# c-zhou/oatk

Hardware: AMD Instinct MI355X
Metric: HiFi Gbases/s through syncasm (syncmer+syncerr) at k=1001 s=31 (higher is better)
Workload: dtype u64

## Files before the change

oatk_amd/csrc/api.hip:

```cpp
#include <hip/hip_runtime.h>
#include <rocprim/device/device_radix_sort.hpp>
#include <rocprim/device/device_scan.hpp>
#include <rocprim/device/device_transform.hpp>
#include <stdio.h>
#include <stdlib.h>
#include <string.h>
#include <time.h>
#include <execinfo.h>
#include <sys/mman.h>
#include <condition_variable>
#include <mutex>
#include <string>
#include <thread>
#include <utility>
#include <vector>

#include "../../include/oatk_hip.h"
#include "common.hpp"
#include "scan_hpc.hpp"
#include "scan_syncmer.hpp"
#include "scan_syncmer_fast.hpp"
#include "kmer_hash.hpp"
#include "count.hpp"

// ... 412 lines not shown
oatk_hip_ctx *oatk_hip_create(int device)
{
    int n = 0;
    if (hipGetDeviceCount(&n) != hipSuccess || device < 0 || device >= n) return nullptr;
    if (hipSetDevice(device) != hipSuccess) return nullptr;
    oatk_hip_ctx *ctx = new oatk_hip_ctx();
    ctx->device = device;
    { int cu = 0; if (hipDeviceGetAttribute(&cu, hipDeviceAttributeMultiprocessorCount, device) == hipSuccess && cu > 0) ctx->n_cu = cu; }
    if (hipStreamCreateWithFlags(&ctx->stream, hipStreamNonBlocking) != hipSuccess) { delete ctx; return nullptr; }
    for (int i = 0; i <= OATK_T_COUNT_; ++i) {
        (void) hipEventCreate(&ctx->ev[i][0]);
        (void) hipEventCreate(&ctx->ev[i][1]);
        ctx->ev_used[i] = false;
    }
    memset(ctx->ms, 0, sizeof(ctx->ms));
    return ctx;
}

void oatk_hip_destroy(oatk_hip_ctx *ctx)
{
    if (!ctx) return;
    (void) hipSetDevice(ctx->device);
    (void) hipStreamSynchronize(ctx->stream);
    DevBuf *all[] = {&ctx->in_seq, &ctx->in_off, &ctx->in_len, &ctx->hoco_l, &ctx->n_scm, &ctx->n_nn, &ctx->n_lrl, &ctx->ho_rl,
                     &ctx->hoco_s, &ctx->nbits, &ctx->nn_key, &ctx->lrl_key, &ctx->lrl_val, &ctx->nn_key2, &ctx->lrl_key2,
                     &ctx->lrl_val2, &ctx->raw_lo, &ctx->raw_smer, &ctx->raw_mpos, &ctx->shard_cnt, &ctx->counters, &ctx->n_scm64,
                     &ctx->scm_off, &ctx->pos_hash, &ctx->pos_lo, &ctx->pos_smer, &ctx->pos_mpos, &ctx->pos_kid, &ctx->key_hash,
                     &ctx->key_sorted, &ctx->iota, &ctx->perm, &ctx->head, &ctx->head_idx, &ctx->newclus, &ctx->clus_id, &ctx->kloc, &ctx->smer_sorted, &ctx->slot_rec, &ctx->scm_loc,
                     &ctx->bad_head, &ctx->tag, &ctx->tmp_perm, &ctx->flags, &ctx->scm_h, &ctx->scm_s, &ctx->scm_cov,
                     &ctx->scm_occ_off, &ctx->scm_occ, &ctx->tmp};
    for (DevBuf *b : all) b->release();
    ec_state_free(ctx);
    cons_state_free(ctx);
    ing_state_free(ctx);
    stat_state_free(ctx);
    ag_state_free(ctx);
    ovl_state_free(ctx);
    ra_state_free(ctx);
    rc_state_free(ctx);
    multi_state_free(ctx);
    for (int i = 0; i <= OATK_T_COUNT_; ++i) {
        (void) hipEventDestroy(ctx->ev[i][0]);
        (void) hipEventDestroy(ctx->ev[i][1]);
    }
    staging_free(ctx);
    (void) hipStreamDestroy(ctx->stream);
    delete ctx;
}

int oatk_hip_mem_pool(oatk_hip_ctx *ctx, uint64_t warm_bytes)
{
    if (!ctx) return OATK_E_NODEV;
    { const char *e = getenv("OATK_POOL"); if (e && e[0] == '0') return OATK_OK; }
    CK(hipSetDevice(ctx->device));
    if (ctx->device < 0 || ctx->device >= 64) return OATK_E_ARG;
    ChunkPool *pl;
    {
        std::unique_lock<std::mutex> lk(g_pool_mu);
        pl = g_pool[ctx->device];
        if (!pl) {
            int vmm = 0;
            if (hipDeviceGetAttribute(&vmm, hipDeviceAttributeVirtualMemoryManagementSupported, ctx->device) != hipSuccess || !vmm) { (void) hipGetLastError(); return OATK_OK; }
            pl = new ChunkPool();
            pl->device = ctx->device;
            memset(&pl->prop, 0, sizeof(pl->prop));
            pl->prop.type = hipMemAllocationTypePinned;
            pl->prop.location.type = hipMemLocationTypeDevice;
            pl->prop.location.id = ctx->device;
            memset(&pl->acc, 0, sizeof(pl->acc));
            pl->acc.location = pl->prop.location;
            pl->acc.flags = hipMemAccessFlagsProtReadWrite;
            static bool at_exit = false;
            if (!at_exit) { at_exit = true; atexit(pools_end); }
            pl->on = true;
            g_pool[ctx->device] = pl;
        }
    }
    if (warm_bytes) pl->warm((size_t) warm_bytes);
    return OATK_OK;
}

const char *oatk_hip_last_error(oatk_hip_ctx *ctx) { return ctx? ctx->err.c_str() : "no device context"; }
void *oatk_hip_stream(oatk_hip_ctx *ctx) { return ctx? (void *) ctx->stream : nullptr; }
int oatk_hip_sync(oatk_hip_ctx *ctx)
{
    if (!ctx) return OATK_E_NODEV;
    CK(hipStreamSynchronize(ctx->stream));
    return OATK_OK;
}
int oatk_hip_set_timing(oatk_hip_ctx *ctx, int enable)
{
    if (!ctx) return OATK_E_NODEV;
    ctx->timing = enable != 0;
    return OATK_OK;
}
int oatk_hip_get_timing(oatk_hip_ctx *ctx, float *ms, int n)
{
    if (!ctx) return OATK_E_NODEV;
    for (int i = 0; i < n && i < OATK_T_COUNT_; ++i) ms[i] = ctx->ms[i];
    return OATK_OK;
}
int oatk_hip_debug_force_general(oatk_hip_ctx *ctx, int on)
{
    if (!ctx) return OATK_E_NODEV;
    ctx->force_general = on != 0;
    return OATK_OK;
}
int oatk_hip_debug_align_two_pass(oatk_hip_ctx *ctx, int on)
{
    if (!ctx) return OATK_E_NODEV;
    ctx->ra_two_pass = on != 0;
    return OATK_OK;
}
int oatk_hip_debug_list_cap(oatk_hip_ctx *ctx, int cap)
{
    if (!ctx) return OATK_E_NODEV;
    if (cap < 0 || cap > oatk::SYF_LIST) { ctx->err = "oatk_hip_debug_list_cap: 0 <= cap <= 128"; return OATK_E_ARG; }
    ctx->list_cap = cap;
    return OATK_OK;
}
int oatk_hip_debug_hash_mask(oatk_hip_ctx *ctx, uint64_t mask)
{
    if (!ctx) return OATK_E_NODEV;
    ctx->hash_mask = mask;
    return OATK_OK;
}

__global__ void widen_kernel(const uint32_t *in, uint64_t *out, uint64_t n)
{
    uint64_t i = (uint64_t) blockIdx.x * blockDim.x + threadIdx.x;
    if (i < n) out[i] = in[i];
    if (i == n) out[i] = 0;
}

static void scan_reset_downstream(oatk_hip_ctx *ctx);

static int launch_scan_kernels(oatk_hip_ctx *ctx)
{
    using namespace oatk;
    const uint64_t n = ctx->n_reads;
    CK(hipMemsetAsync(ctx->counters.p, 0, 4 * sizeof(uint32_t), ctx->stream));
    CK(hipMemsetAsync(ctx->shard_cnt.p, 0, oatk::OATK_REC_SHARDS * sizeof(uint32_t), ctx->stream));
    HpcArgs h;
    h.seq = ctx->d_seq, h.off = ctx->d_off, h.len = ctx->d_len, h.sid0 = ctx->sid0;
    h.ho_rl = ctx->ho_rl.as<uint8_t>(), h.hoco_s = ctx->hoco_s.as<uint8_t>(), h.nbits = ctx->nbits.as<uint32_t>();
    h.hoco_l = ctx->hoco_l.as<uint32_t>(), h.n_nn = ctx->n_nn.as<uint32_t>(), h.n_lrl = ctx->n_lrl.as<uint32_t>();
    h.nn_key = ctx->nn_key.as<uint64_t>(), h.lrl_key = ctx->lrl_key.as<uint64_t>(), h.lrl_val = ctx->lrl_val.as<uint32_t>();
    h.nn_cap = ctx->nn_cap, h.lrl_cap = ctx->lrl_cap, h.counters = ctx->counters.as<uint32_t>();
    t_begin(ctx, OATK_T_HPC);
    h.n_reads = (uint32_t) n;
    constexpr int HPC_NW = 4;
    uint64_t hpc_grid = (uint64_t) ctx->n_cu * 8 * 8;
    { const char *ev = getenv("OATK_DEBUG_HPC_GRID"); if (ev && atoi(ev) > 0) hpc_grid = (uint64_t) atoi(ev); }
    if (hpc_grid * HPC_NW > n) hpc_grid = (n + HPC_NW - 1) / HPC_NW;
    unsigned hpc_dyn = 0;
    { const char *ev = getenv("OATK_DEBUG_HPC_LDS"); if (ev && atoi(ev) > 0) hpc_dyn = (unsigned) atoi(ev); }
    hipLaunchKernelGGL((hpc_pack_kernel<HPC_NW>), dim3((unsigned) (hpc_grid? hpc_grid : 1)), dim3(HPC_NW * OATK_WAVE), hpc_dyn, ctx->stream, h);
    t_end(ctx, OATK_T_HPC);

    SynArgs s;
    s.hoco_s = ctx->hoco_s.as<uint8_t>(), s.nbits = ctx->nbits.as<uint32_t>(), s.off = ctx->d_off;
    s.hoco_l = ctx->hoco_l.as<uint32_t>(), s.n_nn = ctx->n_nn.as<uint32_t>(), s.sid0 = ctx->sid0;
    s.K = ctx->K, s.S = ctx->S, s.want_n = 0, s.n_scm = ctx->n_scm.as<uint32_t>(), s.list_cap = ctx->list_cap? ctx->list_cap : SYF_LIST;
    s.rec_hash = nullptr, s.rec_lo = ctx->raw_lo.as<uint64_t>(), s.rec_smer = ctx->raw_smer.as<uint64_t>();
    s.rec_mpos = ctx->raw_mpos.as<uint32_t>(), s.region_cap = ctx->region_cap, s.shard_cnt = ctx->shard_cnt.as<uint32_t>();
    const bool small = ctx->K + 8 * SYN_NT + 8 + 64 <= 4096;
    const int fast_ring = ctx->force_general? 0 : syncmer_fast_ring(ctx->K, ctx->S);
    t_begin(ctx, OATK_T_SYNCMER);
    if (fast_ring == 4096) {
        const dim3 g((unsigned) n), b(SYN_NT);
        unsigned dyn = 0;
        { const char *ev = getenv("OATK_DEBUG_SYNCMER_LDS"); if (ev && atoi(ev) > 0) dyn = (unsigned) atoi(ev); }
#define OATK_SYF_SWITCH(S31) switch ((-(ctx->K - ctx->S)) & 7) { \
            case 0: OATK_SYF_LAUNCH(S31, 0); break; case 1: OATK_SYF_LAUNCH(S31, 1); break; case 2: OATK_SYF_LAUNCH(S31, 2); break; \
            case 3: OATK_SYF_LAUNCH(S31, 3); break; case 4: OATK_SYF_LAUNCH(S31, 4); break; case 5: OATK_SYF_LAUNCH(S31, 5); break; \
            case 6: OATK_SYF_LAUNCH(S31, 6); break; default: OATK_SYF_LAUNCH(S31, 7); break; }
        const bool two_waves = ctx->K - ctx->S < 1024 && getenv("OATK_DEBUG_SYNCMER_NT256") == nullptr;
#define OATK_SYF_LAUNCH(S31, SH) do { if (two_waves) hipLaunchKernelGGL((syncmer_fast_kernel<2048, S31, 128, SH>), g, dim3(128), dyn, ctx->stream, s); \
                                      else hipLaunchKernelGGL((syncmer_fast_kernel<4096, S31, SYN_NT, SH>), g, b, dyn, ctx->stream, s); } while (0)
        if (ctx->S == 31) OATK_SYF_SWITCH(true) else OATK_SYF_SWITCH(false)
#undef OATK_SYF_SWITCH
#undef OATK_SYF_LAUNCH
    }
    else if (small) hipLaunchKernelGGL((syncmer_kernel<8, 4096, false>), dim3((unsigned) n), dim3(SYN_NT), 0, ctx->stream, s);
    else hipLaunchKernelGGL((syncmer_kernel<16, 8192, false>), dim3((unsigned) n), dim3(SYN_NT), 0, ctx->stream, s);
    t_end(ctx, OATK_T_SYNCMER);
    uint32_t n_amb = 0;
    CK(hipMemcpyAsync(&n_amb, ctx->counters.as<uint32_t>(), 4, hipMemcpyDeviceToHost, ctx->stream));
    CK(hipStreamSynchronize(ctx->stream));
    s.want_n = 1;
    t_begin(ctx, OATK_T_SYNCMER_N);
    if (n_amb) {
        if (small) hipLaunchKernelGGL((syncmer_kernel<8, 4096, true>), dim3((unsigned) n), dim3(SYN_NT), 0, ctx->stream, s);
        else hipLaunchKernelGGL((syncmer_kernel<16, 8192, true>), dim3((unsigned) n), dim3(SYN_NT), 0, ctx->stream, s);
    }
    t_end(ctx, OATK_T_SYNCMER_N);
    CK(hipGetLastError());
    return OATK_OK;
}

int oatk_hip_scan(oatk_hip_ctx *ctx, const uint8_t *d_seq, const uint64_t *d_off, const uint32_t *d_len,
                  uint64_t n_reads, uint64_t seq_bytes, uint64_t sid0, int k, int s)
{
    if (!ctx) return OATK_E_NODEV;
    CK(hipSetDevice(ctx->device));
    if (!(s > 0 && s < 32 && k > s) || k > oatk_hip_max_k()) { ctx->err = "k/s out of range for the device scan"; return OATK_E_ARG; }
    if (seq_bytes % OATK_READ_ALIGN || n_reads >= 0xFFFFFFFFULL || sid0 + n_reads > 0xFFFFFFFFULL) { ctx->err = "bad batch geometry"; return OATK_E_ARG; }
    ctx->d_seq = d_seq, ctx->d_off = d_off, ctx->d_len = d_len;
    ctx->n_reads = n_reads, ctx->seq_bytes = seq_bytes, ctx->sid0 = sid0, ctx->K = k, ctx->S = s;
    scan_reset_downstream(ctx);
    ctx->retries = 0, ctx->collisions = 0;
    ctx->n_occ = ctx->tot_nn = ctx->tot_lrl = ctx->n_scm_total = 0;
    if (n_reads == 0) { ctx->scanned = true; return OATK_OK; }

    ENSURE(hoco_l, n_reads * 4); ENSURE(n_scm, n_reads * 4); ENSURE(n_nn, n_reads * 4); ENSURE(n_lrl, n_reads * 4);
    ENSURE(ho_rl, seq_bytes + 64);
    ENSURE(hoco_s, seq_bytes / 4 + 128 + 16 + ctx->import_reserve);
    ENSURE(nbits, seq_bytes / 8 + 128, true);
    ENSURE(counters, 64);
    if (ctx->nn_cap == 0) ctx->nn_cap = 1u << 14;
    if (ctx->lrl_cap == 0) ctx->lrl_cap = 1u << 14;
    const uint32_t NSH = oatk::OATK_REC_SHARDS;
    {
        uint64_t guess = (seq_bytes / 256 + 1024) / NSH + 256;
        if (ctx->region_cap < guess) ctx->region_cap = (uint32_t) guess;
    }
    ENSURE(shard_cnt, NSH * 4);
    uint32_t sc[oatk::OATK_REC_SHARDS];
    uint32_t sc_max = 0;

    for (;;) {
        const size_t raw_n = (size_t) ctx->region_cap * NSH;
        ENSURE(raw_lo, raw_n * 8); ENSURE(raw_smer, raw_n * 8); ENSURE(raw_mpos, raw_n * 4);
        ENSURE(nn_key, (size_t) ctx->nn_cap * 8); ENSURE(nn_key2, (size_t) ctx->nn_cap * 8);
        ENSURE(lrl_key, (size_t) ctx->lrl_cap * 8); ENSURE(lrl_key2, (size_t) ctx->lrl_cap * 8);
        ENSURE(lrl_val, (size_t) ctx->lrl_cap * 4); ENSURE(lrl_val2, (size_t) ctx->lrl_cap * 4);
        int rc = launch_scan_kernels(ctx);
        if (rc) return rc;
        uint32_t c[4];
        CK(hipMemcpyAsync(c, ctx->counters.p, sizeof(c), hipMemcpyDeviceToHost, ctx->stream));
        CK(hipMemcpyAsync(sc, ctx->shard_cnt.p, sizeof(sc), hipMemcpyDeviceToHost, ctx->stream));
        CK(hipStreamSynchronize(ctx->stream));
        bool again = false;
        if (c[0] > ctx->nn_cap) ctx->nn_cap = c[0] + c[0] / 4, again = true;
        if (c[1] > ctx->lrl_cap) ctx->lrl_cap = c[1] + c[1] / 4, again = true;
        uint64_t tot = 0;
        uint32_t mx = 0;
        for (uint32_t i = 0; i < NSH; ++i) { tot += sc[i]; if (sc[i] > mx) mx = sc[i]; }
        sc_max = mx;
        if (mx > ctx->region_cap) ctx->region_cap = mx + mx / 4 + 16, again = true;
        if (tot > 0xFFFFFFF0ULL) { ctx->err = "more than 2^32 syncmer occurrences in one batch"; return OATK_E_ARG; }
        ctx->tot_nn = c[0], ctx->tot_lrl = c[1], ctx->n_occ = tot;
        if (!again) break;
        ++ctx->retries;
        CK(hipMemsetAsync(ctx->nbits.p, 0, ctx->nbits.cap, ctx->stream));
    }
    if (ctx->timing) t_collect(ctx, OATK_T_HPC, OATK_T_SYNCMER_N);

    t_begin(ctx, OATK_T_SCAN_POST);
    ctx->nn_sorted_in_2 = ctx->lrl_sorted_in_2 = false;
    if (ctx->tot_nn > 1) {
        size_t tb = 0;
        CK(rocprim::radix_sort_keys(nullptr, tb, ctx->nn_key.as<uint64_t>(), ctx->nn_key2.as<uint64_t>(), ctx->tot_nn, 0, 64, ctx->stream));
        ENSURE(tmp, tb);
        CK(rocprim::radix_sort_keys(ctx->tmp.p, tb, ctx->nn_key.as<uint64_t>(), ctx->nn_key2.as<uint64_t>(), ctx->tot_nn, 0, 64, ctx->stream));
        ctx->nn_sorted_in_2 = true;
    }
    if (ctx->tot_lrl > 1) {
        size_t tb = 0;
        CK(rocprim::radix_sort_pairs(nullptr, tb, ctx->lrl_key.as<uint64_t>(), ctx->lrl_key2.as<uint64_t>(), ctx->lrl_val.as<uint32_t>(),
                                     ctx->lrl_val2.as<uint32_t>(), ctx->tot_lrl, 0, 64, ctx->stream));
        ENSURE(tmp, tb);
        CK(rocprim::radix_sort_pairs(ctx->tmp.p, tb, ctx->lrl_key.as<uint64_t>(), ctx->lrl_key2.as<uint64_t>(), ctx->lrl_val.as<uint32_t>(),
                                     ctx->lrl_val2.as<uint32_t>(), ctx->tot_lrl, 0, 64, ctx->stream));
        ctx->lrl_sorted_in_2 = true;
    }
    {
        ENSURE(n_scm64, (n_reads + 1) * 8); ENSURE(scm_off, (n_reads + 1) * 8);
        unsigned nb = (unsigned) ((n_reads + 1 + 255) / 256);
        hipLaunchKernelGGL(widen_kernel, dim3(nb), dim3(256), 0, ctx->stream, ctx->n_scm.as<uint32_t>(), ctx->n_scm64.as<uint64_t>(), n_reads);
        size_t tb = 0;
        CK(rocprim::exclusive_scan(nullptr, tb, ctx->n_scm64.as<uint64_t>(), ctx->scm_off.as<uint64_t>(), (uint64_t) 0, n_reads + 1,
                                   rocprim::plus<uint64_t>(), ctx->stream));
        ENSURE(tmp, tb);
        CK(rocprim::exclusive_scan(ctx->tmp.p, tb, ctx->n_scm64.as<uint64_t>(), ctx->scm_off.as<uint64_t>(), (uint64_t) 0, n_reads + 1,
                                   rocprim::plus<uint64_t>(), ctx->stream));
    }
    t_end(ctx, OATK_T_SCAN_POST);

    {
        size_t n = ctx->n_occ? ctx->n_occ : 1;
        ENSURE(pos_hash, n * 8); ENSURE(pos_lo, n * 8); ENSURE(pos_smer, n * 8); ENSURE(pos_mpos, n * 4);
        ENSURE(key_hash, n * 8); ENSURE(iota, n * 4); ENSURE(slot_rec, n * 32);
    }
    if (ctx->n_occ) {
        oatk::KmerHashArgs kh;
        kh.hoco_s = ctx->hoco_s.as<uint8_t>(), kh.off = ctx->d_off, kh.sid0 = ctx->sid0;
        kh.raw_lo = ctx->raw_lo.as<uint64_t>(), kh.raw_smer = ctx->raw_smer.as<uint64_t>(), kh.raw_mpos = ctx->raw_mpos.as<uint32_t>();
        kh.shard_cnt = ctx->shard_cnt.as<uint32_t>(), kh.region_cap = ctx->region_cap;
        kh.scm_off = ctx->scm_off.as<uint64_t>(), kh.hash_mask = ctx->hash_mask;
        kh.pos_hash = ctx->pos_hash.as<uint64_t>(), kh.pos_lo = ctx->pos_lo.as<uint64_t>(), kh.pos_smer = ctx->pos_smer.as<uint64_t>();
        kh.pos_mpos = ctx->pos_mpos.as<uint32_t>(), kh.key_hash = ctx->key_hash.as<uint64_t>(), kh.iota = ctx->iota.as<uint32_t>();
        kh.slot_rec = ctx->slot_rec.as<uint4>(), kh.K = ctx->K;
        const int nw = ((ctx->K - 1) / 4 + 1 + 7) / 8;
        t_begin(ctx, OATK_T_KMER_HASH);
        hipLaunchKernelGGL(oatk::kmer_hash_kernel, dim3((sc_max + KMH_REC - 1) / KMH_REC, NSH), dim3(64), (size_t) KMH_REC * (nw + 1) * 8, ctx->stream, kh);
        t_end(ctx, OATK_T_KMER_HASH);
    }
    CK(hipGetLastError());
    CK(hipStreamSynchronize(ctx->stream));
    if (ctx->timing) { t_collect(ctx, OATK_T_SCAN_POST, OATK_T_COUNT_PLACE); t_collect(ctx, OATK_T_KMER_HASH, OATK_T_KMER_HASH); }
    ctx->scanned = true;
    ctx->slots_packed = ctx->n_occ != 0;
    return OATK_OK;
}

__global__ void append_rebase_kernel(const uint64_t *src, uint64_t *dst, uint64_t n, uint64_t add)
{
    uint64_t i = (uint64_t) blockIdx.x * blockDim.x + threadIdx.x;
    if (i < n) dst[i] = src[i] + add;
}
__global__ void append_iota_kernel(uint32_t *iota, uint64_t first, uint64_t n)
{
    uint64_t i = (uint64_t) blockIdx.x * blockDim.x + threadIdx.x;
    if (i < n) iota[first + i] = (uint32_t) (first + i);
}

static void scan_reset_downstream(oatk_hip_ctx *ctx)
{
    ctx->scanned = ctx->counted = false;
    ctx->slots_packed = false;
    if (ctx->ec) ctx->ec->done = ctx->ec->marked = ctx->ec->graph_resident = ctx->ec->global = false;
    if (ctx->cons) ctx->cons->done = false;
    if (ctx->ag) ctx->ag->done = false;
    if (ctx->ovl) ctx->ovl->done = false;
    if (ctx->ra) ctx->ra->done = false;
    if (ctx->multi) ctx->multi->merged = ctx->multi->ec_done = false;
}

int oatk_hip_device(oatk_hip_ctx *ctx) { return ctx? ctx->device : -1; }

int oatk_hip_d2d(oatk_hip_ctx *ctx, void *d_dst, const void *d_src, uint64_t bytes)
{
    if (!ctx) return OATK_E_NODEV;
    if (bytes == 0) return OATK_OK;
    CK(hipSetDevice(ctx->device));
    CK(hipMemcpyAsync(d_dst, d_src, bytes, hipMemcpyDeviceToDevice, ctx->stream));
    CK(hipStreamSynchronize(ctx->stream));
    return OATK_OK;
}

int oatk_hip_scan_begin(oatk_hip_ctx *ctx, uint64_t sid0, int k, int s)
{
    if (!ctx) return OATK_E_NODEV;
    CK(hipSetDevice(ctx->device));
    if (!(s > 0 && s < 32 && k > s) || k > oatk_hip_max_k()) { ctx->err = "k/s out of range for the device scan"; return OATK_E_ARG; }
    scan_reset_downstream(ctx);
    ctx->d_seq = nullptr, ctx->d_off = nullptr, ctx->d_len = nullptr;
    ctx->n_reads = 0, ctx->seq_bytes = 0, ctx->sid0 = sid0, ctx->K = k, ctx->S = s;
    ctx->retries = 0, ctx->collisions = 0;
    ctx->n_occ = ctx->tot_nn = ctx->tot_lrl = ctx->n_scm_total = 0;
    ctx->nn_sorted_in_2 = ctx->lrl_sorted_in_2 = false;
    ctx->scanned = true;
    return OATK_OK;
}

#define KEEP(buf, bytes, used)                                                                     \
    do {                                                                                           \
        if (!ctx->buf.grow_keep((bytes), (used), ctx->stream)) {                                   \
            ctx->err = "hipMalloc failed for " #buf " (append)";                                   \
            return OATK_E_NOMEM;                                                                   \
        }                                                                                          \
    } while (0)

static int append_ensure(oatk_hip_ctx *ctx, uint64_t nr, uint64_t sb, uint64_t occ, uint64_t nn, uint64_t lrl)
{
    const uint64_t n0 = ctx->n_reads, b0 = ctx->seq_bytes, o0 = ctx->n_occ;
    KEEP(in_off, (nr + 1) * 8, n0 * 8);
    KEEP(hoco_l, nr * 4 + 4, n0 * 4); KEEP(n_scm, nr * 4 + 4, n0 * 4); KEEP(n_nn, nr * 4 + 4, n0 * 4); KEEP(n_lrl, nr * 4 + 4, n0 * 4);
    KEEP(ho_rl, sb + 64, b0);
    KEEP(hoco_s, sb / 4 + 128 + 16 + ctx->import_reserve, b0 / 4 + 64);
    KEEP(scm_off, (nr + 1) * 8, (n0 + 1) * 8);
    KEEP(pos_hash, occ * 8 + 8, o0 * 8); KEEP(pos_lo, occ * 8 + 8, o0 * 8); KEEP(pos_smer, occ * 8 + 8, o0 * 8); KEEP(pos_mpos, occ * 4 + 4, o0 * 4);
    KEEP(key_hash, occ * 8 + 8, o0 * 8); KEEP(iota, occ * 4 + 4, o0 * 4);
    KEEP(nn_key, nn * 8 + 8, ctx->tot_nn * 8); KEEP(lrl_key, lrl * 8 + 8, ctx->tot_lrl * 8); KEEP(lrl_val, lrl * 4 + 4, ctx->tot_lrl * 4);
    return OATK_OK;
}

int oatk_hip_scan_reserve(oatk_hip_ctx *ctx, uint64_t seq_bytes, uint64_t n_reads, uint64_t n_occ)
{
    if (!ctx) return OATK_E_NODEV;
    CK(hipSetDevice(ctx->device));
    if (!ctx->scanned || ctx->d_seq) { ctx->err = "oatk_hip_scan_reserve: call oatk_hip_scan_begin first"; return OATK_E_STATE; }
    seq_bytes = (seq_bytes + 63) & ~63ULL;
    if (pool_of_current_device()) {
        const uint64_t sb = ctx->seq_bytes + seq_bytes;
        if (!ctx->ho_rl.reserve(sb + 64, ctx->seq_bytes, ctx->stream) || !ctx->hoco_s.reserve(sb / 4 + 128 + 16 + ctx->import_reserve, ctx->seq_bytes / 4 + 64, ctx->stream)) {
            ctx->err = "oatk_hip_scan_reserve: no address range for the batch";
            return OATK_E_NOMEM;
        }
        return OATK_OK;
    }
    return append_ensure(ctx, ctx->n_reads + n_reads, ctx->seq_bytes + seq_bytes, ctx->n_occ + n_occ, ctx->tot_nn, ctx->tot_lrl);
}

int oatk_hip_scan_append(oatk_hip_ctx *ctx, oatk_hip_ctx *src)
{
    if (!ctx || !src) return OATK_E_NODEV;
    CK(hipSetDevice(ctx->device));
    if (ctx == src || ctx->device != src->device) { ctx->err = "oatk_hip_scan_append: the piece must be another handle on the same device"; return OATK_E_ARG; }
    if (!ctx->scanned || ctx->d_seq) { ctx->err = "oatk_hip_scan_append: call oatk_hip_scan_begin first"; return OATK_E_STATE; }
    if (!src->scanned) { ctx->err = "oatk_hip_scan_append: the piece holds no scan"; return OATK_E_STATE; }
    const uint64_t n0 = ctx->n_reads, n1 = src->n_reads, b0 = ctx->seq_bytes, b1 = src->seq_bytes, o0 = ctx->n_occ, o1 = src->n_occ;
    if (n1 == 0) return OATK_OK;
    if (src->K != ctx->K || src->S != ctx->S) { ctx->err = "oatk_hip_scan_append: the piece was scanned with another k / s"; return OATK_E_ARG; }
    if (src->sid0 != ctx->sid0 + n0) { ctx->err = "oatk_hip_scan_append: the piece's first read id must continue the batch"; return OATK_E_ARG; }
    if (n0 + n1 >= 0xFFFFFFFFULL || o0 + o1 > 0xFFFFFFF0ULL) { ctx->err = "oatk_hip_scan_append: batch too large"; return OATK_E_ARG; }
    scan_reset_downstream(ctx);
    ctx->scanned = true;
    { int rc = append_ensure(ctx, n0 + n1, b0 + b1, o0 + o1, ctx->tot_nn + src->tot_nn, ctx->tot_lrl + src->tot_lrl); if (rc) return rc; }
    if (hipStreamSynchronize(src->stream) != hipSuccess) { ctx->err = "oatk_hip_scan_append: the piece's stream failed"; return OATK_E_NODEV; }
    hipStream_t st = ctx->stream;
    auto blocks = [](uint64_t n) { return dim3((unsigned) ((n + 255) / 256 > 0? (n + 255) / 256 : 1)); };
    auto d2d = [&](void *dst, const void *from, size_t bytes) { return bytes? hipMemcpyAsync(dst, from, bytes, hipMemcpyDeviceToDevice, st) : hipSuccess; };
    CK(d2d(ctx->ho_rl.as<uint8_t>() + b0, src->ho_rl.p, b1));
    CK(d2d(ctx->hoco_s.as<uint8_t>() + b0 / 4, src->hoco_s.p, b1 / 4 + 64));
    CK(d2d(ctx->hoco_l.as<uint32_t>() + n0, src->hoco_l.p, n1 * 4)); CK(d2d(ctx->n_scm.as<uint32_t>() + n0, src->n_scm.p, n1 * 4));
    CK(d2d(ctx->n_nn.as<uint32_t>() + n0, src->n_nn.p, n1 * 4)); CK(d2d(ctx->n_lrl.as<uint32_t>() + n0, src->n_lrl.p, n1 * 4));
    hipLaunchKernelGGL(append_rebase_kernel, blocks(n1), dim3(256), 0, st, src->d_off, ctx->in_off.as<uint64_t>() + n0, n1, b0);
    hipLaunchKernelGGL(append_rebase_kernel, blocks(n1 + 1), dim3(256), 0, st, src->scm_off.as<uint64_t>(), ctx->scm_off.as<uint64_t>() + n0, n1 + 1, o0);
    if (o1) {
        CK(d2d(ctx->pos_hash.as<uint64_t>() + o0, src->pos_hash.p, o1 * 8)); CK(d2d(ctx->pos_lo.as<uint64_t>() + o0, src->pos_lo.p, o1 * 8));
        CK(d2d(ctx->pos_smer.as<uint64_t>() + o0, src->pos_smer.p, o1 * 8)); CK(d2d(ctx->pos_mpos.as<uint32_t>() + o0, src->pos_mpos.p, o1 * 4));
        CK(d2d(ctx->key_hash.as<uint64_t>() + o0, src->key_hash.p, o1 * 8));
        hipLaunchKernelGGL(append_iota_kernel, blocks(o1), dim3(256), 0, st, ctx->iota.as<uint32_t>(), o0, o1);
    }
    CK(d2d(ctx->nn_key.as<uint64_t>() + ctx->tot_nn, src->nn_sorted_in_2? src->nn_key2.p : src->nn_key.p, src->tot_nn * 8));
    CK(d2d(ctx->lrl_key.as<uint64_t>() + ctx->tot_lrl, src->lrl_sorted_in_2? src->lrl_key2.p : src->lrl_key.p, src->tot_lrl * 8));
    CK(d2d(ctx->lrl_val.as<uint32_t>() + ctx->tot_lrl, src->lrl_sorted_in_2? src->lrl_val2.p : src->lrl_val.p, src->tot_lrl * 4));
    CK(hipGetLastError());
    CK(hipStreamSynchronize(st));
    ctx->d_off = ctx->in_off.as<uint64_t>();
    ctx->n_reads = n0 + n1, ctx->seq_bytes = b0 + b1, ctx->n_occ = o0 + o1;
    ctx->tot_nn += src->tot_nn, ctx->tot_lrl += src->tot_lrl;
    ctx->retries += src->retries;
    return OATK_OK;
}

int oatk_hip_scan_host(oatk_hip_ctx *ctx, const uint8_t *h_seq, const uint64_t *h_off, const uint32_t *h_len,
                       uint64_t n_reads, uint64_t seq_bytes, uint64_t sid0, int k, int s)
{
    if (!ctx) return OATK_E_NODEV;
    CK(hipSetDevice(ctx->device));
    ENSURE(in_seq, seq_bytes + 64); ENSURE(in_off, (n_reads + 1) * 8); ENSURE(in_len, (n_reads + 1) * 4);
    if (seq_bytes) CK(hipMemcpyAsync(ctx->in_seq.p, h_seq, seq_bytes, hipMemcpyHostToDevice, ctx->stream));
    if (n_reads) {
        CK(hipMemcpyAsync(ctx->in_off.p, h_off, n_reads * 8, hipMemcpyHostToDevice, ctx->stream));
        CK(hipMemcpyAsync(ctx->in_len.p, h_len, n_reads * 4, hipMemcpyHostToDevice, ctx->stream));
    }
    return oatk_hip_scan(ctx, ctx->in_seq.as<uint8_t>(), ctx->in_off.as<uint64_t>(), ctx->in_len.as<uint32_t>(), n_reads, seq_bytes, sid0, k, s);
}

int oatk_hip_count(oatk_hip_ctx *ctx)
{
    using namespace oatk;
    if (!ctx) return OATK_E_NODEV;
    if (!ctx->scanned) { ctx->err = "count before scan"; return OATK_E_STATE; }
    CK(hipSetDevice(ctx->device));
    ctx->counted = false;
    ctx->n_scm_total = 0;
    if (ctx->multi) ctx->multi->merged = ctx->multi->ec_done = false;
    const uint64_t n = ctx->n_occ;
    if (n == 0) { ctx->counted = true; return OATK_OK; }
    const unsigned nb = (unsigned) ((n + 255) / 256);

    ENSURE(key_sorted, n * 8); ENSURE(perm, n * 4); ENSURE(head, n * 4); ENSURE(head_idx, n * 4); ENSURE(newclus, n * 4); ENSURE(kloc, n * 8);
    if (ctx->seq_bytes >> 4 >= 0xFFFFFFFFULL) { ctx->err = "batch too large for 32-bit hoco word indices (64 GB of bases)"; return OATK_E_ARG; }
    ENSURE(clus_id, n * 4); ENSURE(bad_head, n * 4); ENSURE(tag, n * 4); ENSURE(tmp_perm, n * 4); ENSURE(flags, 64);
    ENSURE(pos_kid, n * 8); ENSURE(scm_occ, n * 8);
    CK(hipMemsetAsync(ctx->flags.p, 0, 64, ctx->stream));

    bool full_sort = getenv("OATK_DEBUG_FULL_SORT") != nullptr || n < (1ull << 22);
sort_again:
    t_begin(ctx, OATK_T_COUNT_SORT);
    {
        const unsigned lo_bit = full_sort? 0u : (unsigned) OATK_SORT_LOW_BITS;
        size_t tb = 0;
        CK(rocprim::radix_sort_pairs(nullptr, tb, ctx->key_hash.as<uint64_t>(), ctx->key_sorted.as<uint64_t>(), ctx->iota.as<uint32_t>(),
                                     ctx->perm.as<uint32_t>(), n, lo_bit, 64, ctx->stream));
        ENSURE(tmp, tb);
        CK(rocprim::radix_sort_pairs(ctx->tmp.p, tb, ctx->key_hash.as<uint64_t>(), ctx->key_sorted.as<uint64_t>(), ctx->iota.as<uint32_t>(),
                                     ctx->perm.as<uint32_t>(), n, lo_bit, 64, ctx->stream));
        if (!full_sort) {
            uint32_t *owner = ctx->head.as<uint32_t>();
            CK(hipMemsetAsync(owner, 0xFF, n * 4, ctx->stream));
            hipLaunchKernelGGL(sort_repair_find_kernel, dim3(nb), dim3(256), 0, ctx->stream, ctx->key_sorted.as<uint64_t>(), (uint32_t) n, owner, ctx->flags.as<uint32_t>());
            hipLaunchKernelGGL(sort_repair_kernel, dim3(nb), dim3(256), 0, ctx->stream, ctx->key_sorted.as<uint64_t>(), ctx->perm.as<uint32_t>(), (uint32_t) n, owner,
                               ctx->flags.as<uint32_t>());
        }
    }
    t_end(ctx, OATK_T_COUNT_SORT);

    t_begin(ctx, OATK_T_COUNT_GROUP);
    GroupArgs g;
    g.sorted_key = ctx->key_sorted.as<uint64_t>(), g.perm = ctx->perm.as<uint32_t>(), g.n_rec = (uint32_t) n;
    g.pos_lo = ctx->pos_lo.as<uint64_t>(), g.pos_mpos = ctx->pos_mpos.as<uint32_t>(), g.hoco_s = ctx->hoco_s.as<uint8_t>();
    g.off = ctx->d_off, g.sid0 = ctx->sid0, g.K = ctx->K;
    g.head = ctx->head.as<uint32_t>(), g.head_idx = ctx->head_idx.as<uint32_t>(), g.newclus = ctx->newclus.as<uint32_t>();
    g.loc = ctx->kloc.as<uint64_t>();
    ENSURE(smer_sorted, n * 8);
    g.pos_smer = ctx->pos_smer.as<uint64_t>(), g.occ_sorted = ctx->scm_occ.as<uint64_t>(), g.smer_sorted = ctx->smer_sorted.as<uint64_t>();
    g.flags = ctx->flags.as<uint32_t>();
    ENSURE(slot_rec, n * 32);
    g.slot_rec = ctx->slot_rec.as<uint4>();
    if (!ctx->slots_packed) {
        hipLaunchKernelGGL(pack_slots_kernel, dim3(nb), dim3(256), 0, ctx->stream, g);
        ctx->slots_packed = true;
    }
    hipLaunchKernelGGL((pair_sum_kernel<false>), dim3(2048), dim3(256), 0, ctx->stream, ctx->key_hash.as<uint64_t>(), (const uint32_t *) nullptr, (uint32_t) n, ctx->flags.as<uint32_t>(), 8,
                       (uint32_t *) nullptr, (uint32_t *) nullptr, (uint32_t *) nullptr);
    hipLaunchKernelGGL((pair_sum_kernel<true>), dim3(2048), dim3(256), 0, ctx->stream, ctx->key_sorted.as<uint64_t>(), ctx->perm.as<uint32_t>(), (uint32_t) n, ctx->flags.as<uint32_t>(), 12,
                       g.head, g.newclus, g.head_idx);
    {
        size_t tb = 0;
        CK(rocprim::inclusive_scan(nullptr, tb, ctx->head_idx.as<uint32_t>(), ctx->head_idx.as<uint32_t>(), n, rocprim::maximum<uint32_t>(), ctx->stream));
        ENSURE(tmp, tb);
        CK(rocprim::inclusive_scan(ctx->tmp.p, tb, ctx->head_idx.as<uint32_t>(), ctx->head_idx.as<uint32_t>(), n, rocprim::maximum<uint32_t>(), ctx->stream));
    }
    uint32_t n_scm = 0;
    FinishArgs f;
    auto ids = [&]() -> int {
        size_t tb = 0;
        CK(rocprim::inclusive_scan(nullptr, tb, ctx->newclus.as<uint32_t>(), ctx->clus_id.as<uint32_t>(), n, rocprim::plus<uint32_t>(), ctx->stream));
        ENSURE(tmp, tb);
        CK(rocprim::inclusive_scan(ctx->tmp.p, tb, ctx->newclus.as<uint32_t>(), ctx->clus_id.as<uint32_t>(), n, rocprim::plus<uint32_t>(), ctx->stream));
        uint32_t last_id = 0;
        CK(hipMemcpyAsync(&last_id, ctx->clus_id.as<uint32_t>() + (n - 1), 4, hipMemcpyDeviceToHost, ctx->stream));
        CK(hipStreamSynchronize(ctx->stream));
        n_scm = last_id;
        ENSURE(scm_h, (size_t) n_scm * 8); ENSURE(scm_s, (size_t) n_scm * 8); ENSURE(scm_cov, (size_t) n_scm * 4); ENSURE(scm_loc, (size_t) n_scm * 8);
        ENSURE(scm_occ_off, ((size_t) n_scm + 1) * 8);
        f.perm = ctx->perm.as<uint32_t>(), f.newclus = ctx->newclus.as<uint32_t>(), f.clus_id1 = ctx->clus_id.as<uint32_t>(), f.n_rec = (uint32_t) n;
        f.sorted_key = ctx->key_sorted.as<uint64_t>(), f.smer_sorted = ctx->smer_sorted.as<uint64_t>();
        f.loc = ctx->kloc.as<uint64_t>(), f.scm_loc = ctx->scm_loc.as<uint64_t>();
        f.scm_h = ctx->scm_h.as<uint64_t>(), f.scm_s = ctx->scm_s.as<uint64_t>(), f.scm_occ_off = ctx->scm_occ_off.as<uint64_t>();
        f.scm_occ = ctx->scm_occ.as<uint64_t>(), f.pos_kid = ctx->pos_kid.as<uint64_t>(), f.flags = ctx->flags.as<uint32_t>();
        return OATK_OK;
    };
    { int rc = ids(); if (rc) return rc; }
    hipLaunchKernelGGL(gather_finish_kernel, dim3(nb), dim3(256), 0, ctx->stream, g, f, ctx->clus_id.as<uint32_t>(), n_scm);
    CK(hipMemsetAsync(ctx->bad_head.p, 0, n * 4, ctx->stream));
    hipLaunchKernelGGL(verify_group_kernel, dim3((unsigned) ((n + 8 * OATK_VG_STRIP - 1) / (8 * OATK_VG_STRIP))), dim3(256), 0, ctx->stream, g, ctx->bad_head.as<uint32_t>());
    uint32_t fl[16];
    CK(hipMemcpyAsync(fl, ctx->flags.p, sizeof(fl), hipMemcpyDeviceToHost, ctx->stream));
    CK(hipStreamSynchronize(ctx->stream));
    const bool sort_bad = fl[4] != 0 || memcmp(fl + 8, fl + 12, 16) != 0 || (!full_sort && getenv("OATK_DEBUG_SORT_DISTRUST") != nullptr);
    if (sort_bad && full_sort) {
        t_end(ctx, OATK_T_COUNT_GROUP);
        ctx->err = "the device sort returned something that is not its input in order (rocPRIM radix_sort_pairs): refusing to build the syncmer table from it";
        return OATK_E_NODEV;
    }
    if ((fl[3] || sort_bad) && !full_sort) {
        t_end(ctx, OATK_T_COUNT_GROUP);
        CK(hipMemsetAsync(ctx->flags.p, 0, 64, ctx->stream));
        full_sort = true;
        goto sort_again;
    }
    if (fl[0]) {
        ctx->collisions = 1;
        hipLaunchKernelGGL(split_collisions_kernel, dim3(nb), dim3(256), 0, ctx->stream, g, ctx->bad_head.as<uint32_t>(), ctx->perm.as<uint32_t>(),
                           ctx->tag.as<uint32_t>(), ctx->tmp_perm.as<uint32_t>());
        hipLaunchKernelGGL(regather_kernel, dim3(nb), dim3(256), 0, ctx->stream, g);
        { int rc = ids(); if (rc) return rc; }
        hipLaunchKernelGGL(finish_heads_kernel, dim3(nb), dim3(256), 0, ctx->stream, f, n_scm);
    }
    hipLaunchKernelGGL(check_smer_kernel, dim3(nb), dim3(256), 0, ctx->stream, f);
    hipLaunchKernelGGL(cov_kernel, dim3((n_scm + 255) / 256), dim3(256), 0, ctx->stream, ctx->scm_occ_off.as<uint64_t>(), ctx->scm_cov.as<uint32_t>(), n_scm);
    t_end(ctx, OATK_T_COUNT_GROUP);
    CK(hipGetLastError());
    CK(hipMemcpyAsync(fl, ctx->flags.p, sizeof(fl), hipMemcpyDeviceToHost, ctx->stream));
    CK(hipStreamSynchronize(ctx->stream));
    if (ctx->timing) t_collect(ctx, OATK_T_COUNT_SORT, OATK_T_COUNT_GROUP);
    if (fl[2]) { ctx->err = "hash group with too many distinct k-mers"; return OATK_E_SPLIT; }
    if (debug_refuse(ctx, 4, "oatk_hip_count")) return OATK_E_SPLIT;
    if (fl[1]) { ctx->err = "identical kmers have different smers"; return OATK_E_SMER; }
    ctx->n_scm_total = n_scm;
    ctx->counted = true;
    return OATK_OK;
}

int oatk_hip_info(oatk_hip_ctx *ctx, oatk_hip_info_t *out)
{
    if (!ctx) return OATK_E_NODEV;
    out->n_reads = ctx->n_reads, out->seq_bytes = ctx->seq_bytes, out->sid0 = ctx->sid0;
    out->k = ctx->K, out->s = ctx->S;
    out->n_occ = ctx->n_occ, out->n_nn = ctx->tot_nn, out->n_lrl = ctx->tot_lrl;
    out->n_scm = ctx->n_scm_total;
    out->scan_retries = ctx->retries, out->collisions = ctx->collisions;
    return OATK_OK;
}

int oatk_hip_buffer(oatk_hip_ctx *ctx, int which, const void **d_ptr, uint64_t *bytes)
{
    if (!ctx) return OATK_E_NODEV;
    if (which >= OATK_BUF_INGEST_SEQ && which <= OATK_BUF_INGEST_HDR) return ing_buffer(ctx, which, d_ptr, bytes);
    if (which >= OATK_BUF_MG_H && which <= OATK_BUF_MG_LCOV) return multi_buffer(ctx, which, d_ptr, bytes);
    if (which >= OATK_BUF_MG_G_H && which <= OATK_BUF_MG_POS_GKID) return multi_tail_buffer(ctx, which, d_ptr, bytes);
    if (!ctx->scanned) { ctx->err = "no resident scan"; return OATK_E_STATE; }
    const uint64_t n = ctx->n_reads, occ = ctx->n_occ, ns = ctx->n_scm_total;
// ... 112 lines not shown
```

oatk_amd/csrc/kmer_hash.hpp:

```cpp
#pragma once
#include "common.hpp"
#include "count.hpp"

namespace oatk {

struct KmerHashArgs {
    const uint8_t *hoco_s;
    const uint64_t *off;
    uint64_t sid0;
    const uint64_t *raw_lo;
    const uint64_t *raw_smer;
    const uint32_t *raw_mpos;
    const uint32_t *shard_cnt;
    uint32_t region_cap;
    const uint64_t *scm_off;
    uint64_t hash_mask;
    uint64_t *pos_hash, *pos_lo, *pos_smer;
    uint32_t *pos_mpos;
    uint64_t *key_hash;
    uint32_t *iota;
    uint4 *slot_rec;
    int K;
};

#define KMH_REC 16
#define KMH_WPL 8

__device__ __forceinline__ uint32_t kmh_rev_in_bytes(uint32_t x)
{
    x = ((x >> 2) & 0x33333333u) | ((x & 0x33333333u) << 2);
    return ((x >> 4) & 0x0F0F0F0Fu) | ((x & 0x0F0F0F0Fu) << 4);
}

#ifndef OATK_KMH_WAVES
#define OATK_KMH_WAVES 8
#endif
__global__ __launch_bounds__(64, OATK_KMH_WAVES) void kmer_hash_kernel(KmerHashArgs a)
{
    extern __shared__ uint64_t kmix[];
    const uint32_t lane = threadIdx.x, rr = lane >> 2, q = lane & 3u;
    const uint32_t base = blockIdx.x * (uint32_t) KMH_REC;
    uint32_t cnt = a.shard_cnt[blockIdx.y];
    cnt = cnt < a.region_cap? cnt : a.region_cap;
    if (base >= cnt) return;
    const size_t src = (size_t) blockIdx.y * a.region_cap + base;
    const int K = a.K;
    const int nbytes = (K - 1) / 4 + 1, nfull = nbytes >> 3, nrem = nbytes & 7, NW = nfull + (nrem? 1 : 0);
    const int stride = NW + 1;
    const uint32_t nrec = cnt - base < (uint32_t) KMH_REC? cnt - base : (uint32_t) KMH_REC;
    uint64_t lo = 0;
    uint32_t mp = 0, hsw32 = 0;
    if (rr < nrec) {
        mp = a.raw_mpos[src + rr], lo = a.raw_lo[src + rr];
        const uint32_t rev = mp & 1u, pos = mp >> 1;
        const int64_t hsw = (int64_t) (a.off[(lo >> 32) - a.sid0] >> 4);
        hsw32 = (uint32_t) hsw;
        const uint32_t *hs32 = (const uint32_t *) a.hoco_s;
        uint64_t *out = &kmix[rr * (uint32_t) stride];
        const int per = (NW + 3) >> 2;
        for (int w0 = (int) q * per; w0 < (int) (q + 1) * per && w0 < NW; w0 += KMH_WPL) {
            const int nwd = (int) (q + 1) * per - w0 < KMH_WPL? (int) (q + 1) * per - w0 : KMH_WPL;
            const int n = w0 + nwd > NW? NW - w0 : nwd;
            const int32_t t_lo = rev? (int32_t) pos + K - 32 * (w0 + n) : (int32_t) pos + 32 * w0;
            const int32_t wi = t_lo >> 4;
            const uint32_t sh = ((uint32_t) t_lo & 15u) * 2u;
            uint32_t asc[2 * KMH_WPL + 1];
            const int64_t gbase = hsw + wi;
            if (n == KMH_WPL && gbase >= 0) {
                struct __attribute__((packed, aligned(4))) W4 { uint32_t a, b, c, e; };
                const W4 *src = (const W4 *) (hs32 + gbase);
                const W4 v0 = src[0], v1 = src[1], v2 = src[2], v3 = src[3];
                const uint32_t v4 = hs32[gbase + 16];
                const uint32_t raw[17] = {v0.a, v0.b, v0.c, v0.e, v1.a, v1.b, v1.c, v1.e, v2.a, v2.b, v2.c, v2.e, v3.a, v3.b, v3.c, v3.e, v4};
#pragma unroll
                for (int i = 0; i < 17; ++i) asc[i] = __builtin_bswap32(raw[i]);
            } else {
#pragma unroll
                for (int i = 0; i < 2 * KMH_WPL + 1; ++i) {
                    int64_t gi = gbase + i;
                    gi = gi < 0? 0 : gi;
                    asc[i] = i < 2 * n + 1? __builtin_bswap32(hs32[gi]) : 0u;
                }
            }
#pragma unroll
            for (int c = 0; c < KMH_WPL; ++c) {
                if (c >= n) break;
                const uint32_t x0 = asc[2 * c], x1 = asc[2 * c + 1], x2 = asc[2 * c + 2];
                const uint32_t hi = (uint32_t) (((uint64_t) x0 << 32 | x1) >> (32u - sh));
                const uint32_t lo = (uint32_t) (((uint64_t) x1 << 32 | x2) >> (32u - sh));
                const int j = rev? n - 1 - c : c;
                const int wd = w0 + j;
                int nb = K - 32 * wd;
                nb = nb > 32? 32 : nb;
                uint64_t word;
                if (rev) {
                    uint64_t V = (uint64_t) hi << 32 | lo;
                    if (nb < 32) V &= ~0ULL >> (64 - 2 * nb);
                    const uint64_t R = revcomp32(V);
                    word = nb < 32? bswap64(R & (~0ULL << (64 - 2 * nb)))
                                  : ~((uint64_t) kmh_rev_in_bytes(hi) << 32 | kmh_rev_in_bytes(lo));
                } else {
                    uint64_t V = (uint64_t) hi << 32 | lo;
                    if (nb < 32) V &= ~0ULL << (64 - 2 * nb);
                    word = bswap64(V);
                }
                out[wd] = wd < nfull? murmur_mix_word(word) : word;
            }
        }
    }
    const int from = (int) (lane & 15u) * 4;
    const uint64_t my_lo = (uint64_t) (uint32_t) __shfl((int) (lo >> 32), from) << 32 | (uint32_t) __shfl((int) lo, from);
    const uint32_t my_mp = (uint32_t) __shfl((int) mp, from), my_hsw = (uint32_t) __shfl((int) hsw32, from);
    uint64_t my_p = 0, my_sm = 0;
    if (lane < nrec) my_p = a.scm_off[(my_lo >> 32) - a.sid0] + ((uint32_t) my_lo >> 1), my_sm = a.raw_smer[src + lane];
    __syncthreads();
    if (lane < nrec) {
        const uint64_t *km = &kmix[lane * (uint32_t) stride];
        uint64_t h = OATK_MURMUR_SEED ^ ((uint64_t) (uint32_t) nbytes * OATK_MURMUR_M);
        for (int wd = 0; wd < nfull; ++wd) h = (h ^ km[wd]) * OATK_MURMUR_M;
        if (nrem) h = (h ^ km[nfull]) * OATK_MURMUR_M;
        h ^= h >> 47; h *= OATK_MURMUR_M; h ^= h >> 47;
        a.pos_hash[my_p] = h, a.key_hash[my_p] = h & a.hash_mask;
        a.pos_lo[my_p] = my_lo, a.pos_smer[my_p] = my_sm, a.pos_mpos[my_p] = my_mp, a.iota[my_p] = (uint32_t) my_p;
        a.slot_rec[2 * (size_t) my_p] = make_uint4((uint32_t) my_lo, (uint32_t) (my_lo >> 32), (uint32_t) my_sm, (uint32_t) (my_sm >> 32));
        a.slot_rec[2 * (size_t) my_p + 1] = make_uint4(my_mp, my_hsw, 0u, 0u);
    }
}

}
```

Baseline: 363.0.

## Process 64 records per workgroup with four waves and single-wave hash finalize

```diff
diff --git a/oatk_amd/csrc/api.hip b/oatk_amd/csrc/api.hip
--- a/oatk_amd/csrc/api.hip
+++ b/oatk_amd/csrc/api.hip
@@ -738,9 +738,8 @@
         kh.pos_hash = ctx->pos_hash.as<uint64_t>(), kh.pos_lo = ctx->pos_lo.as<uint64_t>(), kh.pos_smer = ctx->pos_smer.as<uint64_t>();
         kh.pos_mpos = ctx->pos_mpos.as<uint32_t>(), kh.key_hash = ctx->key_hash.as<uint64_t>(), kh.iota = ctx->iota.as<uint32_t>();
         kh.slot_rec = ctx->slot_rec.as<uint4>(), kh.K = ctx->K;
-        const int nw = ((ctx->K - 1) / 4 + 1 + 7) / 8;
         t_begin(ctx, OATK_T_KMER_HASH);
-        hipLaunchKernelGGL(oatk::kmer_hash_kernel, dim3((sc_max + KMH_REC - 1) / KMH_REC, NSH), dim3(64), (size_t) KMH_REC * (nw + 1) * 8, ctx->stream, kh);
+        hipLaunchKernelGGL(oatk::kmer_hash_kernel, dim3((sc_max + KMH_WG_REC - 1) / KMH_WG_REC, NSH), dim3(KMH_WG_WAVES * 64), oatk::kmh_lds_bytes(ctx->K), ctx->stream, kh);
         t_end(ctx, OATK_T_KMER_HASH);
     }
     CK(hipGetLastError());
diff --git a/oatk_amd/csrc/kmer_hash.hpp b/oatk_amd/csrc/kmer_hash.hpp
--- a/oatk_amd/csrc/kmer_hash.hpp
+++ b/oatk_amd/csrc/kmer_hash.hpp
@@ -24,6 +24,8 @@
 };
 
 #define KMH_REC 16
+#define KMH_WG_WAVES 4
+#define KMH_WG_REC (KMH_REC * KMH_WG_WAVES)
 #define KMH_WPL 8
 
 __device__ __forceinline__ uint32_t kmh_rev_in_bytes(uint32_t x)
@@ -32,29 +34,36 @@
     return ((x >> 4) & 0x0F0F0F0Fu) | ((x & 0x0F0F0F0Fu) << 4);
 }
 
+__host__ __device__ inline int kmh_lds_stride(int K)
+{
+    const int nbytes = (K - 1) / 4 + 1;
+    return ((nbytes + 7) >> 3) | 1;
+}
+__host__ __device__ inline size_t kmh_lds_bytes(int K) { return (size_t) KMH_WG_REC * kmh_lds_stride(K) * 8; }
+
 #ifndef OATK_KMH_WAVES
 #define OATK_KMH_WAVES 8
 #endif
-__global__ __launch_bounds__(64, OATK_KMH_WAVES) void kmer_hash_kernel(KmerHashArgs a)
+__global__ __launch_bounds__(KMH_WG_WAVES * 64, OATK_KMH_WAVES) void kmer_hash_kernel(KmerHashArgs a)
 {
     extern __shared__ uint64_t kmix[];
-    const uint32_t lane = threadIdx.x, rr = lane >> 2, q = lane & 3u;
-    const uint32_t base = blockIdx.x * (uint32_t) KMH_REC;
+    const uint32_t lane = threadIdx.x & 63u, q = lane & 3u;
+    const uint32_t wave = __builtin_amdgcn_readfirstlane(threadIdx.x >> 6);
+    const uint32_t rr = wave * (uint32_t) KMH_REC + (lane >> 2);
+    const uint32_t base = blockIdx.x * (uint32_t) KMH_WG_REC;
     uint32_t cnt = a.shard_cnt[blockIdx.y];
     cnt = cnt < a.region_cap? cnt : a.region_cap;
     if (base >= cnt) return;
     const size_t src = (size_t) blockIdx.y * a.region_cap + base;
     const int K = a.K;
     const int nbytes = (K - 1) / 4 + 1, nfull = nbytes >> 3, nrem = nbytes & 7, NW = nfull + (nrem? 1 : 0);
-    const int stride = NW + 1;
-    const uint32_t nrec = cnt - base < (uint32_t) KMH_REC? cnt - base : (uint32_t) KMH_REC;
-    uint64_t lo = 0;
-    uint32_t mp = 0, hsw32 = 0;
+    const int stride = kmh_lds_stride(K);
+    const uint32_t nrec = cnt - base < (uint32_t) KMH_WG_REC? cnt - base : (uint32_t) KMH_WG_REC;
     if (rr < nrec) {
-        mp = a.raw_mpos[src + rr], lo = a.raw_lo[src + rr];
+        const uint32_t mp = a.raw_mpos[src + rr];
+        const uint64_t lo = a.raw_lo[src + rr];
         const uint32_t rev = mp & 1u, pos = mp >> 1;
         const int64_t hsw = (int64_t) (a.off[(lo >> 32) - a.sid0] >> 4);
-        hsw32 = (uint32_t) hsw;
         const uint32_t *hs32 = (const uint32_t *) a.hoco_s;
         uint64_t *out = &kmix[rr * (uint32_t) stride];
         const int per = (NW + 3) >> 2;
@@ -108,18 +117,22 @@
             }
         }
     }
-    const int from = (int) (lane & 15u) * 4;
-    const uint64_t my_lo = (uint64_t) (uint32_t) __shfl((int) (lo >> 32), from) << 32 | (uint32_t) __shfl((int) lo, from);
-    const uint32_t my_mp = (uint32_t) __shfl((int) mp, from), my_hsw = (uint32_t) __shfl((int) hsw32, from);
-    uint64_t my_p = 0, my_sm = 0;
-    if (lane < nrec) my_p = a.scm_off[(my_lo >> 32) - a.sid0] + ((uint32_t) my_lo >> 1), my_sm = a.raw_smer[src + lane];
+    const uint32_t mine = lane < nrec? lane : nrec - 1;
+    uint64_t my_lo = 0;
+    if (wave == 0) my_lo = a.raw_lo[src + mine];
     __syncthreads();
+    if (wave != 0) return;
+    const uint64_t my_sm = a.raw_smer[src + mine];
+    const uint32_t my_mp = a.raw_mpos[src + mine];
+    const uint64_t my_off = a.scm_off[(my_lo >> 32) - a.sid0];
+    const uint32_t my_hsw = (uint32_t) (a.off[(my_lo >> 32) - a.sid0] >> 4);
+    const uint64_t *km = &kmix[mine * (uint32_t) stride];
+    uint64_t h = OATK_MURMUR_SEED ^ ((uint64_t) (uint32_t) nbytes * OATK_MURMUR_M);
+    for (int wd = 0; wd < nfull; ++wd) h = (h ^ km[wd]) * OATK_MURMUR_M;
+    if (nrem) h = (h ^ km[nfull]) * OATK_MURMUR_M;
+    h ^= h >> 47; h *= OATK_MURMUR_M; h ^= h >> 47;
     if (lane < nrec) {
-        const uint64_t *km = &kmix[lane * (uint32_t) stride];
-        uint64_t h = OATK_MURMUR_SEED ^ ((uint64_t) (uint32_t) nbytes * OATK_MURMUR_M);
-        for (int wd = 0; wd < nfull; ++wd) h = (h ^ km[wd]) * OATK_MURMUR_M;
-        if (nrem) h = (h ^ km[nfull]) * OATK_MURMUR_M;
-        h ^= h >> 47; h *= OATK_MURMUR_M; h ^= h >> 47;
+        const uint64_t my_p = my_off + ((uint32_t) my_lo >> 1);
         a.pos_hash[my_p] = h, a.key_hash[my_p] = h & a.hash_mask;
         a.pos_lo[my_p] = my_lo, a.pos_smer[my_p] = my_sm, a.pos_mpos[my_p] = my_mp, a.iota[my_p] = (uint32_t) my_p;
         a.slot_rec[2 * (size_t) my_p] = make_uint4((uint32_t) my_lo, (uint32_t) (my_lo >> 32), (uint32_t) my_sm, (uint32_t) (my_sm >> 32));
```

Result: faster. 366.8, median of 6 (+1.0%).
